# CederGroupHub/chgnet

Measured on AMD Instinct MI355X. Metric: structures/s (energy+force+stress) on batched ~50-atom crystals, higher is better.
Workload: dtype f32; 1 GPU; 1024 x LiMnO2 5x1x1 (40 atoms, sigma=0.01 frac perturbation) per GPU, task efs; structures_per_gpu=1024, atoms=40960, directed_bonds=3535504, angles=4125764, bond_graph_nodes=213755, weights=random-init 0.3.0 architecture (tests/golden/weights_seed0.npz), parallelism=structures sharded over 1 GPU(s), RCCL all-gather of energies only, process_group_ranks=1, energies_in_all_gather=1024, comm=none (single rank)

## Files before the change

chgnet_amd/csrc/engine.hip:

```cpp

#include "engine_internal.h"
#include <cstring>

namespace chgh {

template <int UNROLL>
__global__ __launch_bounds__(256) void k_stream_copy(const f32x4* __restrict__ src, f32x4* __restrict__ dst, size_t n) {
  const size_t stride = (size_t)gridDim.x * blockDim.x;
  size_t i = (size_t)blockIdx.x * blockDim.x + threadIdx.x;
  for (; i + (UNROLL - 1) * stride < n; i += UNROLL * stride) {
    f32x4 v[UNROLL];
#pragma unroll
    for (int u = 0; u < UNROLL; ++u) v[u] = __builtin_nontemporal_load(src + i + u * stride);
#pragma unroll
    for (int u = 0; u < UNROLL; ++u) __builtin_nontemporal_store(v[u], dst + i + u * stride);
  }
  for (; i < n; i += stride) dst[i] = src[i];
}

template <bool NT>
__global__ __launch_bounds__(256) void k_stream_copy_seg(const f32x4* __restrict__ src, f32x4* __restrict__ dst, size_t n) {
  constexpr size_t SEG = 1024;
  const size_t nseg = n / SEG;
  for (size_t sgm = blockIdx.x; sgm < nseg; sgm += gridDim.x) {
// ... 202 lines not shown
    const int sa = acquire_arena(eng, b, total);
    if (sa != CHG_OK) { delete b; return sa; }
  }
  carve(b, b->arena, total);
  if (h->atom_off) b->h_atom_off.assign(h->atom_off, h->atom_off + h->n_struct + 1);
  b->h_volume.resize(h->n_struct);
  for (int q = 0; q < h->n_struct; ++q) {
    const float* Lf = h->lattice + 9 * q;
    b->h_volume[q] = Lf[0] * (Lf[4] * Lf[8] - Lf[5] * Lf[7]) + Lf[1] * (Lf[5] * Lf[6] - Lf[3] * Lf[8]) + Lf[2] * (Lf[3] * Lf[7] - Lf[4] * Lf[6]);
  }
  int s = CHG_OK;
  const size_t B = b->B, N = b->N, Ed = b->Ed, Eu = b->Eu, A = b->A, Eb = b->Eb;
#define UP(field, n) if (s == CHG_OK) s = h2d(eng, b->field, h->field, (n), eng->copy_stream)
  UP(z, N); UP(atom_owner, N); UP(atom_off, B + 1); UP(frac, 3 * N); UP(lattice, 9 * B);
  UP(e_center, Ed); UP(e_nbr, Ed); UP(e_d2u, Ed); UP(e_owner, Ed); UP(e_image, 3 * Ed); UP(e_rev, Ed); UP(p_center, Ed); UP(p_nbr, Ed);
  UP(u_u2d, Eu); UP(u_bnode, Eu); UP(bn_und, Eb);
  UP(a_ctr, A); UP(a_b1c, A); UP(a_b2c, A); UP(a_d1, A); UP(a_d2, A);
#undef UP
  b->win_pending = true;
  if (s == CHG_OK && hipStreamSynchronize(eng->copy_stream) != hipSuccess) { eng->err = "chg_batch_upload: sync failed"; s = CHG_EHIP; }
  if (s != CHG_OK) { hipFree(b->arena); delete b; return s; }
  *out = b;
  return CHG_OK;
}

int chg_debug_fetch_i32(chg_engine* eng, chg_batch* b, const char* name, int32_t* dst, int64_t capacity, int64_t* n_written) {
  if (!eng || !b || !name || !dst) return CHG_EINVAL;
  if (std::strcmp(name, "wide_range") == 0) {
    if (capacity >= 1) dst[0] = b->wide_range ? 1 : 0;
    if (n_written) *n_written = capacity >= 1 ? 1 : 0;
    return CHG_OK;
  }
  if (std::strcmp(name, "route") == 0) {
    const int64_t n = std::min<int64_t>(6, std::max<int64_t>(capacity, 0));
    std::copy(b->route, b->route + n, dst);
    if (n_written) *n_written = n;
    return CHG_OK;
  }
  if (b->named_i32.empty()) register_names(b);
  auto it = b->named_i32.find(name);
  if (it == b->named_i32.end()) { eng->err = std::string("chg_debug_fetch_i32: unknown buffer ") + name; return CHG_EINVAL; }
  const size_t n = std::min<size_t>(it->second.second, (size_t)std::max<int64_t>(capacity, 0));
  TRY(ensure_windows(eng, b));
  HIP_TRY(eng, hipStreamSynchronize(eng->stream));
  if (n) HIP_TRY(eng, hipMemcpy(dst, it->second.first, n * sizeof(int32_t), hipMemcpyDeviceToHost));
  if (n_written) *n_written = (int64_t)n;
  return CHG_OK;
}

int chg_batch_update_geometry(chg_engine* eng, chg_batch* b, const float* frac, const float* lattice) {
  if (!eng || !b) return CHG_EINVAL;
  HIP_TRY(eng, hipSetDevice(eng->device));
  int s = CHG_OK;
  if (frac) s = h2d(eng, b->frac, frac, (size_t)3 * b->N);
  if (s == CHG_OK && lattice) {
    s = h2d(eng, b->lattice, lattice, (size_t)9 * b->B);
    b->h_volume.resize(b->B);
    for (int q = 0; q < b->B; ++q) {
      const float* Lf = lattice + 9 * (size_t)q;
      b->h_volume[q] = Lf[0] * (Lf[4] * Lf[8] - Lf[5] * Lf[7]) + Lf[1] * (Lf[5] * Lf[6] - Lf[3] * Lf[8]) + Lf[2] * (Lf[3] * Lf[7] - Lf[4] * Lf[6]);
    }
  }
  b->q_tables = false;
  if (s == CHG_OK) HIP_TRY(eng, hipStreamSynchronize(eng->stream));
  return s;
}

// ... 14 lines not shown
  }
  delete b;
  return CHG_OK;
}

int64_t chg_batch_device_bytes(const chg_batch* b) { return b ? (int64_t)b->arena_bytes : 0; }

int chg_predict(chg_engine* eng, chg_batch* b, uint32_t task_mask) {
  if (!eng || !b) return CHG_EINVAL;
  HIP_TRY(eng, hipSetDevice(eng->device));
  const uint32_t task = task_mask | CHG_TASK_E;
  TRY(ensure_windows(eng, b));
  if (eng->force_wide) b->wide_range = true;
  if (b->wide_range) return chgh_wide::run_predict(eng, b, task);
  if (eng->profiling || !eng->use_graphs) return run_predict(eng, b, task);
  if (b->graph_task != task) {
    if (b->graph_exec) hipGraphExecDestroy(b->graph_exec);
    b->graph_exec = nullptr;
    b->graph_task = task;
    b->eager_calls = 0;
  }
  if (!b->graph_exec && b->eager_calls++ == 0) return run_predict(eng, b, task);
  if (!b->graph_exec) {
    hipGraph_t graph = nullptr;
    HIP_TRY(eng, hipStreamBeginCapture(eng->stream, hipStreamCaptureModeThreadLocal));
    const int s = run_predict(eng, b, task);
    const hipError_t e = hipStreamEndCapture(eng->stream, &graph);
    if (s != CHG_OK) { if (graph) hipGraphDestroy(graph); return s; }
    if (e != hipSuccess) { eng->err = std::string("hipStreamEndCapture: ") + hipGetErrorString(e); return CHG_EHIP; }
    const hipError_t ei = hipGraphInstantiate(&b->graph_exec, graph, nullptr, nullptr, 0);
    hipGraphDestroy(graph);
    if (ei != hipSuccess) { b->graph_exec = nullptr; eng->err = std::string("hipGraphInstantiate: ") + hipGetErrorString(ei); return CHG_EHIP; }
    b->graph_task = task;
    std::copy(b->route, b->route + 6, b->graph_route);
  }
  HIP_TRY(eng, hipGraphLaunch(b->graph_exec, eng->stream));
  std::copy(b->graph_route, b->graph_route + 6, b->route);
  b->last_task = task;
  b->seed1_adjoints = (task & (CHG_TASK_F | CHG_TASK_S)) != 0;
  b->q_tables = b->seed1_adjoints;
  return CHG_OK;
}

int chg_engine_update_weights(chg_engine* eng, const float* weights_blob) {
  if (!eng || !weights_blob) return CHG_EINVAL;
  TRY(check_weight_range(eng, weights_blob, (size_t)eng->desc.n_weights));
  HIP_TRY(eng, hipSetDevice(eng->device));
  HIP_TRY(eng, hipMemcpyAsync(eng->d_weights, weights_blob, sizeof(float) * (size_t)eng->desc.n_weights, hipMemcpyHostToDevice, eng->stream));
  TRY(build_images(eng));
  HIP_TRY(eng, hipStreamSynchronize(eng->stream));
  return CHG_OK;
}

int chg_batch_all_gather_energy(chg_engine* eng, chg_batch* b, chg_comm* comm, int64_t width, float* table) {
  if (!eng || !b || !comm || !table || width < b->B) return CHG_EINVAL;
  if (b->last_task == 0) { eng->err = "chg_batch_all_gather_energy: run chg_predict on this batch first"; return CHG_EINVAL; }
  HIP_TRY(eng, hipSetDevice(eng->device));
  int32_t nranks = 1, comm_dev = -1;
  float* stage = nullptr;
  if (chg_comm_info(comm, nullptr, &nranks, &comm_dev) == CHG_OK && comm_dev != eng->device) {
    eng->err = "chg_batch_all_gather_energy: the communicator belongs to device " + std::to_string(comm_dev) + ", the engine to device " + std::to_string(eng->device);
    return CHG_EINVAL;
  }
  if (chg_comm_info(comm, nullptr, &nranks, nullptr) != CHG_OK || chg_comm_reserve(comm, width * (int64_t)(nranks + 1), &stage) != CHG_OK) {
    eng->err = std::string("chg_batch_all_gather_energy: ") + chg_comm_last_error(comm);
    return CHG_EHIP;
  }
  hipStream_t st = eng->stream;
  HIP_TRY(eng, hipMemsetAsync(stage, 0, sizeof(float) * (size_t)width, st));
  HIP_TRY(eng, hipMemcpyAsync(stage, b->energy, sizeof(float) * (size_t)b->B, hipMemcpyDeviceToDevice, st));
// ... 234 lines not shown
```

chgnet_amd/csrc/engine_internal.h:

```cpp
#pragma once

#include "chgnet_hip.h"

#include <hip/hip_runtime.h>

#include <algorithm>
#include <cmath>
#include <cstdint>
#include <cstdio>
#include <cstdlib>
#include <cstring>
#include <functional>
#include <map>
#include <mutex>
#include <string>
#include <unordered_map>
#include <vector>

#include "mfma_tile.h"
#include "mfma_split.h"
#include "kernels_conv.h"
#include "kernels_angle_w.h"
#include "kernels_angle_blk.h"
#include "kernels_embed.h"
// ... 18 lines not shown
};

struct ErrText {
  static std::unordered_map<const ErrText*, std::string>& texts() {
    thread_local std::unordered_map<const ErrText*, std::string> t;
    return t;
  }
  std::string& slot() const { return texts()[this]; }
  ErrText& operator=(const std::string& v) { slot() = v; return *this; }
  ErrText& operator=(const char* v) { slot() = v; return *this; }
  operator std::string() const { return slot(); }
  const char* c_str() const { return slot().c_str(); }
  ~ErrText() { texts().erase(this); }
};
inline std::string operator+(const char* a, const ErrText& b) { return std::string(a) + std::string(b); }
inline std::string operator+(const std::string& a, const ErrText& b) { return a + std::string(b); }
inline std::string operator+(const ErrText& a, const char* b) { return std::string(a) + b; }
inline std::string operator+(const ErrText& a, const std::string& b) { return std::string(a) + b; }

struct ProfEntry { std::string label; int64_t launches = 0; double ms = 0.0; };
struct PendingEvent { int entry; hipEvent_t start, stop; };

struct chg_engine {
  int device = 0;
  hipStream_t stream = nullptr;
  chg_model_desc desc{};
  float* d_weights = nullptr;
  Weights w{};
  float* d_images = nullptr;
  const float* p_elem = nullptr;
  const float* img_ac_fwd[2][MAX_CONV] = {};
  const float* img_ac_bwd_rm[MAX_CONV] = {};
  const float* img_angle[2][2 * MAX_CONV] = {};
  ErrText err;
  hipEvent_t t0 = nullptr, t1 = nullptr;
  bool profiling = false;
  std::vector<ProfEntry> prof;
  std::map<std::string, int> prof_index;
  std::vector<PendingEvent> pending;
  std::vector<hipEvent_t> event_pool;
  hipStream_t copy_stream = nullptr;
  std::mutex pool_mu;
  std::vector<std::pair<char*, size_t>> arena_pool;
  std::vector<std::pair<char*, size_t>> work_pool;
  std::vector<int> work_kind;
  bool use_graphs = true;
  bool force_wide = false;
  char* scratch = nullptr;
  size_t scratch_bytes = 0, scratch_wanted = 0;
  char* h_stage = nullptr;
  size_t h_stage_bytes = 0;
  char* h_out = nullptr;
  size_t h_out_bytes = 0;
  int num_cus = 256;
  bool spec_builds = true;
  int last_N = 0, last_Ed = 0, last_A = 0, last_Eb = 0;
  double last_r_atom = 0.0, last_r_bond = 0.0;
  long n_spec_builds = 0, n_spec_overflows = 0, n_cell_builds = 0, n_cell_fallbacks = 0;
  int graph_search = 0;
  int cell_min_atoms = 2048;
  size_t memory_limit = 0;
};

struct Train2;

struct chg_batch {
// ... 2 lines not shown
  size_t arena_bytes = 0;
  int *z, *atom_owner, *atom_off, *e_center, *e_nbr, *e_d2u, *e_owner, *e_rev, *p_center, *p_nbr, *u_u2d, *u_bnode, *bn_und, *a_ctr, *a_b1c, *a_b2c, *a_d1, *a_d2;
  float *frac, *lattice, *e_image;
  float* cart;
  f32x4 *ev, *eu;
  float *hb0, *wag, *wbgc;
  float* atom[MAX_CONV + 1];
  float* hbc[MAX_CONV + 1];
  float* ang[MAX_CONV];
  float* Pl[MAX_CONV];
  float* Ql[MAX_CONV];
  float* Rl[2 * MAX_CONV];
  float* Sl[2 * MAX_CONV];
  float* agg_l[MAX_CONV];
  float* aggB_l[MAX_CONV];
  float* GP_l[MAX_CONV];
  float* GR_l[2 * MAX_CONV];
  float* GS_l[2 * MAX_CONV];
  float* zsave_l[2 * MAX_CONV] = {};
  float *energy, *site_energy, *site_raw, *magmom, *crystal_fea, *force, *virial, *volume;
  float *Ga, *GA, *Gb, *Gwag, *Gwbgc, *Gang, *GQ, *Gagg, *Grk, *Gu;
  WinIndex win{};
  int *win_tmp = nullptr, *win_scan = nullptr;
  int win_grid = 64;
  bool win_built = false;
  bool canonical = false;
  bool win_index_ready = false;
  int win_team = 0;
  int blk_cap = 0;
  bool blk_ready = false;
  int *blk_a = nullptr, *blk_b1c = nullptr, *blk_b2c = nullptr, *blk_ctr = nullptr, *blk_desc = nullptr, *blk_tiles = nullptr;
  bool win_pending = false;
  bool zsave_now = false;
  int32_t route[6] = {}, graph_route[6] = {};
  size_t addr_span = 0;
  int p_table_done = -1;
  float *zero1, *zero1_end, *zero2, *zero2_end;
  float* zero2_keep_end = nullptr;
  uint32_t last_task = 0;
  bool seed1_adjoints = false;
  hipGraphExec_t graph_exec = nullptr;
  uint32_t graph_task = 0;
  int eager_calls = 0;
  std::map<std::string, std::pair<const float*, size_t>> named;
  std::map<std::string, std::pair<const int*, size_t>> named_i32;
  char* train_arena = nullptr;
  size_t train_bytes = 0;
  std::vector<int> h_atom_off;
  std::vector<double> h_volume;
  char* t2_arena = nullptr;
  size_t t2_bytes = 0;
  struct Train2* t2 = nullptr;
  float* t_mcot = nullptr;
  float h_g_b3 = 0.f;
  bool q_tables = false;
  bool wide_range = false;
  bool t_has_mcot = false;
  float *t_grad = nullptr, *t_cot = nullptr, *t_tmp = nullptr , *t_dumpG = nullptr, *t_dumpH = nullptr, *t_dumpZ = nullptr, *t_Xb = nullptr, *t_Xa = nullptr,
        *t_ro = nullptr;
};

#define HIP_TRY(eng, expr)                                                                          \
  do {                                                                                              \
    hipError_t _e = (expr);                                                                         \
    if (_e != hipSuccess) {                                                                         \
      (eng)->err = std::string(#expr) + ": " + hipGetErrorString(_e);                               \
      return CHG_EHIP;                                                                              \
// ... 135 lines not shown
```

chgnet_amd/csrc/engine_predict.hip:

```cpp
#include "engine_internal.h"

#include "kernels_geom.h"
#include "kernels_angle_fa.h"
#include "kernels_chain.h"

namespace chgh {


struct Cursor {
  const float* base;
  size_t pos = 0;
  const float* take(size_t n) {
    pos += (4 - pos % 4) % 4;
    const float* p = base + pos;
    pos += n;
    return p;
  }
};

void take_gated_tail(Cursor& c, GatedW& g, const float*& w2c_t, const float*& w2g_t) {
  g.w2c = c.take(D * D); g.b2c = c.take(D); g.w2g = c.take(D * D); g.b2g = c.take(D);
  w2c_t = c.take(D * D); w2g_t = c.take(D * D);
}
void take_ln(Cursor& c, GatedW& g) {
  g.ln1_g = c.take(D); g.ln1_b = c.take(D); g.ln2_g = c.take(D); g.ln2_b = c.take(D);
}

size_t layout_weights(const float* base, int L, Weights& w) {
  Cursor c{base};
  w.atomref = c.take(94); w.emb = c.take(94 * D);
  w.freq_ag = c.take(NRAD); w.freq_bg = c.take(NRAD); w.freq_ang = c.take(NFREQ);
  w.w_bond_emb = c.take(D * NRAD); w.w_wag = c.take(D * NRAD); w.w_wbg = c.take(D * NRAD); w.w_ang_emb = c.take(D * NANG);
  for (int l = 0; l < L; ++l) {
    ACW& a = w.ac[l];
    a.w_cn = c.take(4 * D * D); a.w_bond = c.take(2 * D * D); a.b1 = c.take(2 * D); a.q_bias = c.take(2 * D); a.q_shift = c.take(D);
    take_gated_tail(c, a.g, a.w2c_t, a.w2g_t);
    take_ln(c, a.g);
// ... 137 lines not shown
  hipLaunchKernelGGL((k_rows_gemm_multi<K, SMALL_GEMM_COLS>), dim3(grid_for(m.max_rows, 4 * eng->num_cus), blocks), dim3(BLOCK),
                     (rows_gemm_lds<K, SMALL_GEMM_COLS, (K == 128 ? 2 : 1)>()), eng->stream, m.g);
  HIP_TRY(eng, hipGetLastError());
  return CHG_OK;
}
static bool small_rows(int rows) { return rows > 0 && rows <= SMALL_GEMM_ROWS; }

int zero(chg_engine* eng, void* p, size_t bytes) {
  if (bytes == 0) return CHG_OK;
  LaunchScope ls(eng, "memset");
  HIP_TRY(eng, hipMemsetAsync(p, 0, bytes, eng->stream));
  return CHG_OK;
}





static bool addr32_mode(const chg_batch* b) {
  constexpr size_t HARD = (size_t)1 << 32;
  static const int forced = [] { const char* e = std::getenv("CHGNET_ADDR_MODE"); return e ? std::atoi(e) : 0; }();
  static const size_t limit = [] { const char* e = std::getenv("CHGNET_ADDR32_MAX_BYTES"); return e ? (size_t)std::strtoull(e, nullptr, 10) : HARD; }();
  if (b->addr_span == 0 || b->addr_span >= HARD || forced == 64) return false;
  return forced == 32 || b->addr_span < limit;
}

int build_images(chg_engine* eng) {
  const int L = eng->desc.n_conv;
  constexpr size_t AF = ac_fwd_image_floats(), AB = ac_bwd_rm_image_floats();
  constexpr size_t BF = AngleLds<true, false>::tiles, BB = AngleLds<true, true>::tiles, UF = AngleLds<false, false>::tiles,
                   UB = AngleLds<false, true>::tiles;
  static_assert(AF % 4 == 0 && AB % 4 == 0 && BF % 4 == 0 && BB % 4 == 0 && UF % 4 == 0 && UB % 4 == 0, "images are copied in 16-byte units");
  constexpr size_t PE = (size_t)94 * 4 * D;
  const size_t total = (size_t)L * (2 * AF + AB) + (size_t)(L - 1) * (BF + BB + UF + UB) + PE;
  if (!eng->d_images) {
    HIP_TRY(eng, hipMalloc(&eng->d_images, total * sizeof(float)));
    HIP_TRY(eng, hipMemsetAsync(eng->d_images, 0, total * sizeof(float), eng->stream));
  }
  float* at = eng->d_images;
  auto take = [&](size_t n) { float* p = at; at += n; return p; };
  for (int l = 0; l < L; ++l) {
    AtomConvArgs a{};
    a.gw = eng->w.ac[l].g; a.w_bond = eng->w.ac[l].w_bond;
    for (int qb = 0; qb < 2; ++qb) {
      a.q_bias = qb ? eng->w.ac[l].q_bias : nullptr;
      float* img = take(AF);
      eng->img_ac_fwd[qb][l] = img;
      hipLaunchKernelGGL(k_atomconv_image<>, dim3(1), dim3(BLOCK), 0, eng->stream, a, img);
    }
    float* img = take(AB);
    eng->img_ac_bwd_rm[l] = img;
    hipLaunchKernelGGL(k_atomconv_image_rm, dim3(1), dim3(BLOCK), 0, eng->stream, a, img);
  }
  for (int l = 0; l + 1 < L; ++l) {
    const BCW& bc = eng->w.bc[l];
    const AUW& au = eng->w.au[l];
    float* img;
    eng->img_angle[0][l] = img = take(BF);
    hipLaunchKernelGGL((k_angle_image<true, false>), dim3(1), dim3(BLOCK), 0, eng->stream, bc.w_ang, bc.g, img);
    eng->img_angle[1][l] = img = take(BB);
    hipLaunchKernelGGL((k_angle_image<true, true>), dim3(1), dim3(BLOCK), 0, eng->stream, bc.w_ang, bc.g, img);
    eng->img_angle[0][L + l] = img = take(UF);
    hipLaunchKernelGGL((k_angle_image<false, false>), dim3(1), dim3(BLOCK), 0, eng->stream, au.w_ang, au.g, img);
    eng->img_angle[1][L + l] = img = take(UB);
    hipLaunchKernelGGL((k_angle_image<false, true>), dim3(1), dim3(BLOCK), 0, eng->stream, au.w_ang, au.g, img);
  }
  {
    float* tab = take(PE);
    eng->p_elem = tab;
    const ACW& w0 = eng->w.ac[0];
    TRY(rows_gemm_out2(eng, "gemm_Pelem", eng->w.emb, nullptr, w0.w_cn, w0.w_cn + 2 * D * D, w0.b1, tab, 4 * D, 94));
  }
  HIP_TRY(eng, hipGetLastError());
  return CHG_OK;
}

static bool tiny_batch(const chg_batch* b) {
  static const bool on = [] { const char* e = std::getenv("CHGNET_TINY_FUSE"); return !e || std::atoi(e) != 0; }();
  return on && b->N <= SMALL_GEMM_ROWS && b->Ed <= (1 << 18) && b->A <= (1 << 19);
}

static RowsGemm atomconv_p_problem(chg_engine* eng, chg_batch* b, int l) {
  const ACW& w = eng->w.ac[l];
  return RowsGemm{b->atom[l], D, nullptr, w.w_cn, w.b1, nullptr, 0, b->Pl[l], 4 * D, nullptr, b->N, 0, w.w_cn + 2 * D * D, 0, 2 * D, 0, 0};
}

int atomconv_tables(chg_engine* eng, chg_batch* b, int l) {
  const ACW& w = eng->w.ac[l];
  if (b->p_table_done == l) return CHG_OK;
  return rows_gemm_out2(eng, "gemm_P", b->atom[l], nullptr, w.w_cn, w.w_cn + 2 * D * D, w.b1, b->Pl[l], 4 * D, b->N);
}

int atomconv_q_table(chg_engine* eng, chg_batch* b, int l) {
  const ACW& w = eng->w.ac[l];
  float* Q = b->Ql[l];
  if (b->Eu == 0) return CHG_OK;
  TRY(rows_gemm(eng, "gemm_Q", 64, 128, b->hb0, D, nullptr, w.w_bond, b->A > 0 ? w.q_bias : nullptr, nullptr, 0, Q, 2 * D, nullptr, b->Eu, 0));
  if (b->Eb > 0 && b->hbc[l] != b->hbc[0])
    TRY(rows_gemm(eng, "gemm_Qnode", 64, 128, b->hbc[l], D, nullptr, w.w_bond, nullptr, nullptr, 0, Q, 2 * D, b->bn_und, b->Eb, 0));
  return CHG_OK;
}

AtomConvArgs atomconv_args(chg_engine* eng, chg_batch* b, int l) {
  AtomConvArgs a{};
// ... 312 lines not shown
        cb.term(p, b->GR_l[L + l], 4 * D, nullptr, w.au[l].w_bij_t, 2 * D);
        cb.term(p, b->GR_l[L + l] + 2 * D, 4 * D, nullptr, w.au[l].w_bij_t + 2 * D * D, 2 * D);
        p.Y1 = b->Gb; p.y1_idx = b->bn_und; p.ldy1 = D;
      }
      p.add = b->Gb; p.add_idx = b->bn_und; p.lda = D;
      cb.out(p, w.bc[l].w_out_t, nullptr, b->Gagg, D, D);
      if (au) {
        ChainProb& q = cb.add(b->N);
        cb.term(q, b->GS_l[L + l], 2 * D, nullptr, w.au[l].w_ctr_t, 2 * D);
        q.add = b->Ga; q.lda = D; q.Y1 = b->Ga; q.ldy1 = D;
      }
      TRY(launch_chain(eng, "chain_Bt", cb));
    }
    TRY((launch_angle<true, true>(eng, "bondconv_bwd", b, angle_args(b, l, b->ang[l], w.bc[l].w_ang, w.bc[l].g, nullptr))));
    {
      ChainBuilder cb;
      ChainProb& p = cb.add(b->N);
      cb.term(p, b->GS_l[l], 2 * D, nullptr, w.bc[l].w_ctr_t, 2 * D);
      cb.term(p, b->GP_l[l + 1], 4 * D, nullptr, w.ac[l + 1].w_cn_t, 2 * D);
      cb.term(p, b->GP_l[l + 1] + 2 * D, 4 * D, nullptr, w.ac[l + 1].w_cn_t + 2 * D * D, 2 * D);
      p.add = b->Ga; p.lda = D; p.Y1 = b->Ga; p.ldy1 = D;
      cb.out(p, w.ac[l].w_out_t, nullptr, b->GA, D, D);
      ChainProb& q = cb.add(b->Eb);
      cb.term(q, b->GR_l[l], 4 * D, nullptr, w.bc[l].w_bij_t, 2 * D);
      cb.term(q, b->GR_l[l] + 2 * D, 4 * D, nullptr, w.bc[l].w_bij_t + 2 * D * D, 2 * D);
      q.add = b->Gb; q.add_idx = b->bn_und; q.lda = D; q.Y1 = b->Gb; q.y1_idx = b->bn_und; q.ldy1 = D;
      TRY(launch_chain(eng, "chain_At", cb));
    }
    TRY(atomconv_bwd_kernel(eng, b, l));
  }
  return CHG_OK;
}

int run_predict(chg_engine* eng, chg_batch* b, uint32_t task) {
  const Weights& w = eng->w;
  const int L = b->L;
  const bool want_f = task & CHG_TASK_F, want_s = task & CHG_TASK_S, want_m = task & CHG_TASK_M;
  const bool want_grad = want_f || want_s;
  hipStream_t st = eng->stream;

  const bool tiny = tiny_batch(b);
  b->zsave_now = want_grad;
  const size_t zero_bytes = (size_t)((char*)(want_grad ? b->zero2_end : b->zero1_end) - (char*)b->zero1);
  b->p_table_done = -1;
  if (tiny) {
    PrologueArgs a{};
    a.frac = b->frac; a.lattice = b->lattice; a.atom_owner = b->atom_owner; a.z = b->z; a.n_atoms = b->N;
    a.e_center = b->e_center; a.e_nbr = b->e_nbr; a.e_owner = b->e_owner; a.e_image = b->e_image; a.n_edges = b->Ed;
    a.cart = b->cart; a.ev = b->ev; a.eu = b->eu; a.emb = w.emb; a.atom0 = b->atom[0];
    a.p_elem = b->Ed > 0 ? eng->p_elem : nullptr; a.P0 = b->Pl[0];
    a.zero_begin = reinterpret_cast<f32x4*>(b->zero1); a.zero_n = zero_bytes / sizeof(f32x4);
    LaunchScope ls(eng, "prologue");
    hipLaunchKernelGGL(k_prologue, dim3(std::min<unsigned>(4 * eng->num_cus, g1(std::max<int64_t>(b->Ed, (int64_t)b->N * D)).x)), dim3(256), 0, st, a);
    if (a.p_elem) b->p_table_done = 0;
  } else {
    LaunchScope ls(eng, "cart");
    hipLaunchKernelGGL(k_cart, g1(b->N), dim3(256), 0, st, b->frac, b->lattice, b->atom_owner, b->cart, b->N);
  }
  if (b->Ed > 0) {
    if (!tiny) { LaunchScope ls(eng, "edge_geom");
      hipLaunchKernelGGL(k_edge_geom, g1(b->Ed), dim3(256), 0, st, b->cart, b->lattice, b->e_center, b->e_nbr, b->e_image, b->e_owner, b->ev, b->eu, b->Ed); }
    if (tiny) {
      EmbedAllArgs ea{bond_embed_args(eng, b), angle_embed_args(eng, b), grid_for(b->Eu, 2 * eng->num_cus),
                      b->Eb > 0 ? grid_for(b->Eb, 2 * eng->num_cus) : 0, b->A > 0 ? grid_for(b->A, EMBED_GRID_MULT * eng->num_cus) : 0};
      LaunchScope ls(eng, "embed_fwd");
      hipLaunchKernelGGL(k_embed_all<false>, dim3(ea.g_bond1 + ea.g_bond2 + ea.g_angle), dim3(BLOCK), bond_embed_lds(), st, ea);
    } else { LaunchScope ls(eng, "bond_embed_fwd");
      hipLaunchKernelGGL((k_bond_embed_fwd_o4<1>), dim3(grid_for(b->Eu, 2 * eng->num_cus)), dim3(BLOCK), bond_embed_lds(), st, bond_embed_args(eng, b));
      if (b->Eb > 0)
        hipLaunchKernelGGL((k_bond_embed_t<false, false, 2>), dim3(grid_for(b->Eb, 2 * eng->num_cus)), dim3(BLOCK), bond_embed_lds(), st, bond_embed_args(eng, b)); }
  }
  if (b->A > 0 && !(tiny && b->Ed > 0)) {
    LaunchScope ls(eng, "angle_embed_fwd");
    hipLaunchKernelGGL((k_angle_embed_fwd_o4<0>), dim3(grid_for(b->A, EMBED_GRID_MULT * eng->num_cus)), dim3(BLOCK), angle_embed_lds(), st, angle_embed_args(eng, b));
  }
  if (!tiny) { LaunchScope ls(eng, "atom_embed");
    hipLaunchKernelGGL(k_atom_embed, g1((int64_t)b->N * (D / 4)), dim3(256), 0, st, b->z, w.emb, b->atom[0], b->N); }
  HIP_TRY(eng, hipGetLastError());

  if (!tiny) TRY(zero(eng, b->zero1, zero_bytes));
  static const bool chain_on = [] { const char* e = std::getenv("CHGNET_TINY_CHAIN"); return !e || std::atoi(e) != 0; }();
  const bool chained = tiny && chain_on && L >= 2 && b->Ed > 0 && b->A > 0 && b->Eb > 0 && b->p_table_done == 0;
  b->route[0] = tiny;
  b->route[1] = chained;
  b->route[2] = want_grad && b->zsave_l[0] && (b->win_built || b->win_team > 0);
  b->route[3] = b->win_built;
  b->route[4] = b->win_team > 0;
  b->route[5] = addr32_mode(b);
  if (chained) {
    TRY(forward_tiny(eng, b, want_grad, want_m));
  } else {
  for (int l = 0; l < L - 1; ++l) {
    TRY(atomconv_fwd(eng, b, l, want_grad));
    if (b->A > 0) {
      TRY(bondconv_fwd(eng, b, l));
      if (l < L - 2) TRY(angleupd_fwd(eng, b, l));
    }
  }
  if (want_m) {
    LaunchScope ls(eng, "magmom");
    hipLaunchKernelGGL(k_magmom, dim3(wave_grid(eng, b->N)), dim3(256), 0, st, b->atom[L - 1], w.site_w, w.site_b, b->magmom, b->N);
  }
  TRY(atomconv_fwd(eng, b, L - 1, want_grad));
  }

  {
    ReadoutArgs r{};
    r.atom = b->atom[L]; r.atom_owner = b->atom_owner; r.z = b->z; r.n_atoms = b->N;
    r.ln_g = w.ro_ln_g; r.ln_b = w.ro_ln_b; r.w0 = w.mlp_w0; r.b0 = w.mlp_b0; r.w1 = w.mlp_w1; r.b1 = w.mlp_b1;
    r.w2 = w.mlp_w2; r.b2 = w.mlp_b2; r.w3 = w.mlp_w3; r.b3 = w.mlp_b3; r.atomref = w.atomref;
    r.has_composition = eng->desc.has_composition; r.n_hidden = eng->desc.n_mlp_hidden;
    r.site_energy = b->site_energy; r.site_raw = b->site_raw; r.crystal_fea = b->crystal_fea;
    r.Ga = want_grad ? b->Ga : nullptr;
    const int tiles16 = (b->N + TILE_ROWS - 1) / TILE_ROWS;
    r.wpb = std::max(1, std::min(WAVES, (tiles16 + eng->num_cus - 1) / eng->num_cus));
    LaunchScope ls(eng, "readout");
    hipLaunchKernelGGL(k_readout<false>, dim3(grid_for(b->N, eng->num_cus, r.wpb * TILE_ROWS)), dim3(BLOCK), readout_lds(), st, r);
    HIP_TRY(eng, hipGetLastError());
  }

  if (want_grad) {
    if (chained) {
      TRY(reverse_tiny(eng, b));
    } else {
    TRY(atomconv_bwd(eng, b, L - 1));
    for (int l = L - 2; l >= 0; --l) {
      if (b->A > 0) {
        if (l < L - 2) TRY(angleupd_bwd(eng, b, l));
        TRY(bondconv_bwd(eng, b, l));
      }
      TRY(atomconv_bwd(eng, b, l));
    }
    }
    if (b->Ed > 0) {
      if (tiny) {
        EmbedAllArgs ea{bond_embed_args(eng, b), angle_embed_args(eng, b), grid_for(b->Eu, 2 * eng->num_cus),
                        b->Eb > 0 ? grid_for(b->Eb, 2 * eng->num_cus) : 0, b->A > 0 ? grid_for(b->A, EMBED_GRID_MULT * eng->num_cus) : 0};
        LaunchScope ls(eng, "embed_bwd");
        hipLaunchKernelGGL(k_embed_all<true>, dim3(ea.g_bond1 + ea.g_bond2 + ea.g_angle), dim3(BLOCK), bond_embed_lds(), st, ea);
      } else { LaunchScope ls(eng, "bond_embed_bwd");
        hipLaunchKernelGGL((k_bond_embed_t<true, false, 1>), dim3(grid_for(b->Eu, 2 * eng->num_cus)), dim3(BLOCK), bond_embed_lds(), st, bond_embed_args(eng, b));
        if (b->Eb > 0)
          hipLaunchKernelGGL((k_bond_embed_t<true, false, 2>), dim3(grid_for(b->Eb, 2 * eng->num_cus)), dim3(BLOCK), bond_embed_lds(), st, bond_embed_args(eng, b)); }
      if (b->A > 0 && !tiny) {
        LaunchScope ls(eng, "angle_embed_bwd");
        hipLaunchKernelGGL((k_angle_embed_t<true>), dim3(grid_for(b->A, EMBED_GRID_MULT * eng->num_cus)), dim3(BLOCK), angle_embed_lds(), st, angle_embed_args(eng, b));
      }
      ForceArgs f{};
      f.ev = b->ev; f.eu = b->eu; f.Gu = b->Gu; f.Grk = b->Grk;
      f.e_center = b->e_center; f.e_d2u = b->e_d2u; f.e_owner = b->e_owner; f.e_rev = b->e_rev; f.u_u2d = b->u_u2d;
      f.n_edges = b->Ed; f.force = b->force; f.virial = b->virial;
      LaunchScope ls(eng, "edge_force");
      hipLaunchKernelGGL(k_edge_force, g1(b->Ed, EF_EDGES_PER_BLOCK), dim3(256), 0, st, f);
    }
    HIP_TRY(eng, hipGetLastError());
  }
// ... 211 lines not shown
  if ((s = set_lds(eng, k_rows_gemm<128, SMALL_GEMM_COLS, 2>, (rows_gemm_lds<128, SMALL_GEMM_COLS, 2>())))) return s;
  if ((s = set_lds(eng, (k_rows_gemm<64, 128, 2>), (rows_gemm_lds<64, 128, 2>())))) return s;
  if ((s = set_lds(eng, (k_rows_gemm<128, 64, 2>), (rows_gemm_lds<128, 64, 2>())))) return s;
  if ((s = set_lds(eng, k_atomconv_fwd<FWD_WAVES>, (atomconv_lds<FWD_WAVES, false, true>())))) return s;
  if ((s = set_lds(eng, k_atomconv_bwd<false>, acb_fused_lds()))) return s;
  if ((s = set_lds(eng, k_angleupd_fwd_a<>, angle_fa_lds()))) return s;
  if ((s = set_lds(eng, (k_atomconv_fwd<FWD_WAVES, true>), (atomconv_lds<FWD_WAVES, false, true>())))) return s;
  if ((s = set_lds(eng, (k_atomconv_bwd<false, true>), acb_fused_lds()))) return s;
  if ((s = set_lds(eng, k_angleupd_fwd_a<true>, angle_fa_lds()))) return s;
  if ((s = set_lds(eng, (k_angle_bwd_w<true, false, false, true>), angle_w_lds<true>()))) return s;
  if ((s = set_lds(eng, (k_angle_bwd_w<true, false, true, true>), angle_w_lds<true>()))) return s;
  if ((s = set_lds(eng, (k_angle_bwd_w<false, false, false, true>), angle_w_lds<false>()))) return s;
  if ((s = set_lds(eng, (k_angle<true, false, WAVES, false, true>), angle_lds<true>()))) return s;
  if ((s = set_lds(eng, k_angle_bwd_blk<true>, angle_blk_lds<true>()))) return s;
  if ((s = set_lds(eng, k_angle_bwd_blk<false>, angle_blk_lds<false>()))) return s;
  if ((s = set_lds(eng, k_angle_bwd_w<true>, angle_w_lds<true>()))) return s;
  if ((s = set_lds(eng, k_angle_bwd_w<false>, angle_w_lds<false>()))) return s;
  if ((s = set_lds(eng, (k_angle_bwd_w<true, true>), angle_w_lds<true>()))) return s;
  if ((s = set_lds(eng, (k_angle_bwd_w<true, false, true>), angle_w_lds<true>()))) return s;
  if ((s = set_lds(eng, (k_angle_bwd_w<true, true, true>), angle_w_lds<true>()))) return s;
  if ((s = set_lds(eng, (k_angle_bwd_w<false, true>), angle_w_lds<false>()))) return s;
  if ((s = set_lds(eng, k_angle<true, false>, angle_lds<true>()))) return s;
  if ((s = set_lds(eng, k_angle<true, true>, (angle_lds<true, WAVES, true>())))) return s;
  if ((s = set_lds(eng, k_angle<false, true>, (angle_lds<false, WAVES, true>())))) return s;
  if ((s = set_lds(eng, k_angle<false, false, FWD_WAVES>, (angle_lds<false, FWD_WAVES>())))) return s;
  if ((s = set_lds(eng, k_readout<false>, readout_lds()))) return s;
  if ((s = set_lds(eng, (k_bond_embed_t<false, false, 2>), bond_embed_lds()))) return s;
  if ((s = set_lds(eng, (k_bond_embed_t<true, false, 1>), bond_embed_lds()))) return s;
  if ((s = set_lds(eng, (k_bond_embed_t<true, false, 2>), bond_embed_lds()))) return s;
  if ((s = set_lds(eng, k_angle_embed_fwd_o4<0>, angle_embed_lds()))) return s;
  if ((s = set_lds(eng, k_bond_embed_fwd_o4<1>, bond_embed_lds()))) return s;
  if ((s = set_lds(eng, k_angle_embed_t<true>, angle_embed_lds()))) return s;
  if ((s = set_lds(eng, k_rows_chain, chain_lds()))) return s;
  if ((s = set_lds(eng, k_embed_all<false>, bond_embed_lds()))) return s;
  if ((s = set_lds(eng, k_embed_all<true>, bond_embed_lds()))) return s;
  return CHG_OK;
}


}
```

Measured before the change: 40710 structures/s.

## Merge per-row linear layers into multi-output MFMA kernels for forward and reverse

Result: no change. 40810 structures/s, median of 6 (+0.2%).

```diff
diff --git a/chgnet_amd/csrc/engine.hip b/chgnet_amd/csrc/engine.hip
--- a/chgnet_amd/csrc/engine.hip
+++ b/chgnet_amd/csrc/engine.hip
@@ -258,7 +258,7 @@
     return CHG_OK;
   }
   if (std::strcmp(name, "route") == 0) {
-    const int64_t n = std::min<int64_t>(6, std::max<int64_t>(capacity, 0));
+    const int64_t n = std::min<int64_t>(chg_batch::N_ROUTE, std::max<int64_t>(capacity, 0));
     std::copy(b->route, b->route + n, dst);
     if (n_written) *n_written = n;
     return CHG_OK;
@@ -339,10 +339,10 @@
     hipGraphDestroy(graph);
     if (ei != hipSuccess) { b->graph_exec = nullptr; eng->err = std::string("hipGraphInstantiate: ") + hipGetErrorString(ei); return CHG_EHIP; }
     b->graph_task = task;
-    std::copy(b->route, b->route + 6, b->graph_route);
+    std::copy(b->route, b->route + chg_batch::N_ROUTE, b->graph_route);
   }
   HIP_TRY(eng, hipGraphLaunch(b->graph_exec, eng->stream));
-  std::copy(b->graph_route, b->graph_route + 6, b->route);
+  std::copy(b->graph_route, b->graph_route + chg_batch::N_ROUTE, b->route);
   b->last_task = task;
   b->seed1_adjoints = (task & (CHG_TASK_F | CHG_TASK_S)) != 0;
   b->q_tables = b->seed1_adjoints;
diff --git a/chgnet_amd/csrc/engine_internal.h b/chgnet_amd/csrc/engine_internal.h
--- a/chgnet_amd/csrc/engine_internal.h
+++ b/chgnet_amd/csrc/engine_internal.h
@@ -74,6 +74,8 @@
   const float* img_ac_fwd[2][MAX_CONV] = {};
   const float* img_ac_bwd_rm[MAX_CONV] = {};
   const float* img_angle[2][2 * MAX_CONV] = {};
+  struct RowsImg { const float *cn, *cn_t, *ctr, *ctr_t, *bij, *bij_t, *out, *out_t; };
+  RowsImg img_rows_ac[MAX_CONV] = {}, img_rows_bc[MAX_CONV] = {}, img_rows_au[MAX_CONV] = {};
   ErrText err;
   hipEvent_t t0 = nullptr, t1 = nullptr;
   bool profiling = false;
@@ -142,7 +144,8 @@
   int *blk_a = nullptr, *blk_b1c = nullptr, *blk_b2c = nullptr, *blk_ctr = nullptr, *blk_desc = nullptr, *blk_tiles = nullptr;
   bool win_pending = false;
   bool zsave_now = false;
-  int32_t route[6] = {}, graph_route[6] = {};
+  static constexpr int N_ROUTE = 7;
+  int32_t route[N_ROUTE] = {}, graph_route[N_ROUTE] = {};
   size_t addr_span = 0;
   int p_table_done = -1;
   float *zero1, *zero1_end, *zero2, *zero2_end;
diff --git a/chgnet_amd/csrc/engine_predict.hip b/chgnet_amd/csrc/engine_predict.hip
--- a/chgnet_amd/csrc/engine_predict.hip
+++ b/chgnet_amd/csrc/engine_predict.hip
@@ -3,6 +3,7 @@
 #include "kernels_geom.h"
 #include "kernels_angle_fa.h"
 #include "kernels_chain.h"
+#include "kernels_rows.h"
 
 namespace chgh {
 
@@ -206,7 +207,9 @@
                    UB = AngleLds<false, true>::tiles;
   static_assert(AF % 4 == 0 && AB % 4 == 0 && BF % 4 == 0 && BB % 4 == 0 && UF % 4 == 0 && UB % 4 == 0, "images are copied in 16-byte units");
   constexpr size_t PE = (size_t)94 * 4 * D;
-  const size_t total = (size_t)L * (2 * AF + AB) + (size_t)(L - 1) * (BF + BB + UF + UB) + PE;
+  constexpr size_t RA = 4 * RM_IMG64 + 2 * RM_IMG128 + 2 * RM_IMG64, RU = 2 * RM_IMG64 + RM_IMG128 + 4 * RM_IMG64 + 2 * RM_IMG128,
+                   RB = RU + 2 * RM_IMG64;
+  const size_t total = (size_t)L * (2 * AF + AB) + (size_t)(L - 1) * (BF + BB + UF + UB) + PE + (size_t)L * RA + (size_t)(L - 1) * (RB + RU);
   if (!eng->d_images) {
     HIP_TRY(eng, hipMalloc(&eng->d_images, total * sizeof(float)));
     HIP_TRY(eng, hipMemsetAsync(eng->d_images, 0, total * sizeof(float), eng->stream));
@@ -244,6 +247,31 @@
     eng->p_elem = tab;
     const ACW& w0 = eng->w.ac[0];
     TRY(rows_gemm_out2(eng, "gemm_Pelem", eng->w.emb, nullptr, w0.w_cn, w0.w_cn + 2 * D * D, w0.b1, tab, 4 * D, 94));
+  }
+  {
+    auto images = [&](const float* W, int K, int n) {
+      float* first = take((size_t)n * D * K);
+      for (int q = 0; q < n; ++q)
+        hipLaunchKernelGGL(k_rows_image, dim3(1), dim3(BLOCK), 0, eng->stream, W + (size_t)q * D * K, D, K, first + (size_t)q * D * K);
+      return (const float*)first;
+    };
+    for (int l = 0; l < L; ++l) {
+      const ACW& a = eng->w.ac[l];
+      chg_engine::RowsImg& r = eng->img_rows_ac[l];
+      r = chg_engine::RowsImg{};
+      r.cn = images(a.w_cn, D, 4); r.cn_t = images(a.w_cn_t, 2 * D, 2); r.out = images(a.w_out, D, 1); r.out_t = images(a.w_out_t, D, 1);
+    }
+    for (int l = 0; l + 1 < L; ++l) {
+      const BCW& bc = eng->w.bc[l];
+      const AUW& au = eng->w.au[l];
+      chg_engine::RowsImg& rb = eng->img_rows_bc[l];
+      rb = chg_engine::RowsImg{};
+      rb.ctr = images(bc.w_ctr, D, 2); rb.ctr_t = images(bc.w_ctr_t, 2 * D, 1); rb.bij = images(bc.w_bij, D, 4); rb.bij_t = images(bc.w_bij_t, 2 * D, 2);
+      rb.out = images(bc.w_out, D, 1); rb.out_t = images(bc.w_out_t, D, 1);
+      chg_engine::RowsImg& ru = eng->img_rows_au[l];
+      ru = chg_engine::RowsImg{};
+      ru.ctr = images(au.w_ctr, D, 2); ru.ctr_t = images(au.w_ctr_t, 2 * D, 1); ru.bij = images(au.w_bij, D, 4); ru.bij_t = images(au.w_bij_t, 2 * D, 2);
+    }
   }
   HIP_TRY(eng, hipGetLastError());
   return CHG_OK;
@@ -622,6 +650,149 @@
   return CHG_OK;
 }
 
+static int rows_merge_mode() {
+  static const int mode = [] {
+    const char* e = std::getenv("CHGNET_ROWS_MERGE");
+    const int v = e ? std::atoi(e) : 1;
+    return v == 0 ? 0 : v == 2 ? 1 : v == 3 ? 2 : 3;
+  }();
+  return mode;
+}
+
+struct MergeBuilder {
+  RowsMerge p{};
+  explicit MergeBuilder(int rows) { p.rows = rows; }
+  void term(const float* X, int ldx, const float* img, int K) { p.t[p.nterms++] = ChainTerm{X, nullptr, img, ldx, K}; }
+  void out(const float* img, const float* bias, int bias_blocks, float* Y, int ldy, int nblocks) {
+    for (int q = 0; q < nblocks; ++q)
+      p.o[p.nouts++] = RmOut{img + (size_t)q * RM_IMG64, (bias && q < bias_blocks) ? bias + q * D : nullptr, Y + q * D, ldy};
+  }
+  void add(const float* rows, const int* idx) { p.add = rows; p.idx = idx; p.lda = D; }
+  void store(float* Y1) { p.Y1 = Y1; p.ldy1 = D; }
+};
+
+int launch_rows_merge(chg_engine* eng, const char* label, MergeBuilder& mb) {
+  RowsMerge& p = mb.p;
+  if (p.rows <= 0) return CHG_OK;
+  const int K = p.nterms ? p.t[0].K : D;
+  for (int t = 1; t < p.nterms; ++t)
+    if (p.t[t].K != K) { eng->err = "rows_merge: terms of different widths"; return CHG_EINVAL; }
+  const int ny = (p.nouts + 3) / 4;
+  p.outs_per_block = ny ? (p.nouts + ny - 1) / ny : 0;
+  const size_t lds = rows_merge_lds(p);
+  if (lds > RM_LDS_CAP || (ny > 1 && p.Y1 == p.add)) { eng->err = "rows_merge: unsupported problem"; return CHG_EINVAL; }
+  const int ntiles = (p.rows + BLOCK_ROWS - 1) / BLOCK_ROWS;
+  const int gx = rm_phases(p.nterms) > 1 ? ntiles : grid_for(p.rows, std::max(8, 2 * eng->num_cus / std::max(ny, 1)));
+  LaunchScope ls(eng, label);
+  const dim3 grid(gx, std::max(ny, 1));
+  if (K == D) hipLaunchKernelGGL(k_rows_merge<D>, grid, dim3(BLOCK), lds, eng->stream, p);
+  else hipLaunchKernelGGL(k_rows_merge<2 * D>, grid, dim3(BLOCK), lds, eng->stream, p);
+  HIP_TRY(eng, hipGetLastError());
+  return CHG_OK;
+}
+
+int forward_merged(chg_engine* eng, chg_batch* b, bool want_grad, bool want_m) {
+  const Weights& w = eng->w;
+  const int L = b->L;
+  const bool angles = b->A > 0;
+  for (int l = 0; l < L; ++l) {
+    if (b->p_table_done != l) {
+      MergeBuilder mb(b->N);
+      mb.add(b->atom[l], nullptr);
+      mb.out(eng->img_rows_ac[l].cn, w.ac[l].b1, 2, b->Pl[l], 4 * D, 4);
+      TRY(launch_rows_merge(eng, "rows_atom_f", mb));
+      b->p_table_done = l;
+    }
+    TRY(atomconv_fwd_kernel(eng, b, l, want_grad));
+    {
+      MergeBuilder mb(b->N);
+      mb.term(b->agg_l[l], D, eng->img_rows_ac[l].out, D);
+      mb.p.bias1 = w.ac[l].b_out;
+      mb.add(b->atom[l], nullptr);
+      mb.store(b->atom[l + 1]);
+      if (l < L - 1) {
+        if (angles) mb.out(eng->img_rows_bc[l].ctr, w.bc[l].b1, 2, b->Sl[l], 2 * D, 2);
+        mb.out(eng->img_rows_ac[l + 1].cn, w.ac[l + 1].b1, 2, b->Pl[l + 1], 4 * D, 4);
+        if (angles && l < L - 2) mb.out(eng->img_rows_au[l].ctr, w.au[l].b1, 2, b->Sl[L + l], 2 * D, 2);
+      }
+      TRY(launch_rows_merge(eng, "rows_atom_f", mb));
+      if (l < L - 1) b->p_table_done = l + 1;
+    }
+    if (l == L - 1) break;
+    if (angles) {
+      if (l == 0) {
+        MergeBuilder mb(b->Eb);
+        mb.add(b->hbc[0], nullptr);
+        mb.out(eng->img_rows_bc[0].bij, nullptr, 0, b->Rl[0], 4 * D, 4);
+        TRY(launch_rows_merge(eng, "rows_bond_f", mb));
+      }
+      TRY((launch_angle<true, false>(eng, "bondconv_fwd", b, angle_args(b, l, b->ang[l], w.bc[l].w_ang, w.bc[l].g, b->aggB_l[l]))));
+      MergeBuilder mb(b->Eb);
+      mb.term(b->aggB_l[l], D, eng->img_rows_bc[l].out, D);
+      mb.p.bias1 = w.bc[l].b_out;
+      mb.add(b->hbc[l], nullptr);
+      mb.store(b->hbc[l + 1]);
+      if (l < L - 2) {
+        mb.out(eng->img_rows_au[l].bij, nullptr, 0, b->Rl[L + l], 4 * D, 4);
+        mb.out(eng->img_rows_bc[l + 1].bij, nullptr, 0, b->Rl[l + 1], 4 * D, 4);
+      }
+      TRY(launch_rows_merge(eng, "rows_bond_f", mb));
+      if (l < L - 2)
+        TRY((launch_angle<false, false, FWD_WAVES>(eng, "angleupd_fwd", b, angle_args(b, L + l, b->ang[l], w.au[l].w_ang, w.au[l].g, b->ang[l + 1]))));
+    }
+    if (l == L - 2 && want_m) {
+      LaunchScope ls(eng, "magmom");
+      hipLaunchKernelGGL(k_magmom, dim3(wave_grid(eng, b->N)), dim3(256), 0, eng->stream, b->atom[L - 1], w.site_w, w.site_b, b->magmom, b->N);
+    }
+  }
+  return CHG_OK;
+}
+
+int reverse_merged(chg_engine* eng, chg_batch* b) {
+  const int L = b->L;
+  const bool angles = b->A > 0;
+  auto gr_terms = [&](MergeBuilder& mb, int slot, const chg_engine::RowsImg& im) {
+    mb.term(b->GR_l[slot], 4 * D, im.bij_t, 2 * D);
+    mb.term(b->GR_l[slot] + 2 * D, 4 * D, im.bij_t + RM_IMG128, 2 * D);
+  };
+  for (int l = L - 1; l >= 0; --l) {
+    if (angles && l < L - 1) {
+      const bool au = l < L - 2;
+      if (au) TRY((launch_angle<false, true>(eng, "angleupd_bwd", b, angle_args(b, L + l, b->ang[l], eng->w.au[l].w_ang, eng->w.au[l].g, nullptr))));
+      {
+        MergeBuilder mb(b->Eb);
+        if (au) { gr_terms(mb, L + l, eng->img_rows_au[l]); mb.store(b->Gb); }
+        mb.add(b->Gb, b->bn_und);
+        mb.out(eng->img_rows_bc[l].out_t, nullptr, 0, b->Gagg, D, 1);
+        TRY(launch_rows_merge(eng, "rows_bond_b", mb));
+      }
+      TRY((launch_angle<true, true>(eng, "bondconv_bwd", b, angle_args(b, l, b->ang[l], eng->w.bc[l].w_ang, eng->w.bc[l].g, nullptr))));
+      {
+        MergeBuilder mb(b->Eb);
+        gr_terms(mb, l, eng->img_rows_bc[l]);
+        mb.add(b->Gb, b->bn_und);
+        mb.store(b->Gb);
+        TRY(launch_rows_merge(eng, "rows_bond_b", mb));
+      }
+    }
+    {
+      MergeBuilder mb(b->N);
+      if (l < L - 1) {
+        if (angles && l < L - 2) mb.term(b->GS_l[L + l], 2 * D, eng->img_rows_au[l].ctr_t, 2 * D);
+        if (angles) mb.term(b->GS_l[l], 2 * D, eng->img_rows_bc[l].ctr_t, 2 * D);
+        mb.term(b->GP_l[l + 1], 4 * D, eng->img_rows_ac[l + 1].cn_t, 2 * D);
+        mb.term(b->GP_l[l + 1] + 2 * D, 4 * D, eng->img_rows_ac[l + 1].cn_t + RM_IMG128, 2 * D);
+        mb.store(b->Ga);
+      }
+      mb.add(b->Ga, nullptr);
+      mb.out(eng->img_rows_ac[l].out_t, nullptr, 0, b->GA, D, 1);
+      TRY(launch_rows_merge(eng, "rows_atom_b", mb));
+    }
+    TRY(atomconv_bwd_kernel(eng, b, l));
+  }
+  return CHG_OK;
+}
+
 int run_predict(chg_engine* eng, chg_batch* b, uint32_t task) {
   const Weights& w = eng->w;
   const int L = b->L;
@@ -677,8 +848,12 @@
   b->route[3] = b->win_built;
   b->route[4] = b->win_team > 0;
   b->route[5] = addr32_mode(b);
+  const int merged = (!tiny && L >= 2 && b->Ed > 0) ? rows_merge_mode() : 0;
+  b->route[6] = merged;
   if (chained) {
     TRY(forward_tiny(eng, b, want_grad, want_m));
+  } else if (merged & 1) {
+    TRY(forward_merged(eng, b, want_grad, want_m));
   } else {
   for (int l = 0; l < L - 1; ++l) {
     TRY(atomconv_fwd(eng, b, l, want_grad));
@@ -712,6 +887,8 @@
   if (want_grad) {
     if (chained) {
       TRY(reverse_tiny(eng, b));
+    } else if (merged & 2) {
+      TRY(reverse_merged(eng, b));
     } else {
     TRY(atomconv_bwd(eng, b, L - 1));
     for (int l = L - 2; l >= 0; --l) {
@@ -989,6 +1166,8 @@
   if ((s = set_lds(eng, k_bond_embed_fwd_o4<1>, bond_embed_lds()))) return s;
   if ((s = set_lds(eng, k_angle_embed_t<true>, angle_embed_lds()))) return s;
   if ((s = set_lds(eng, k_rows_chain, chain_lds()))) return s;
+  if ((s = set_lds(eng, k_rows_merge<D>, RM_LDS_CAP))) return s;
+  if ((s = set_lds(eng, k_rows_merge<2 * D>, RM_LDS_CAP))) return s;
   if ((s = set_lds(eng, k_embed_all<false>, bond_embed_lds()))) return s;
   if ((s = set_lds(eng, k_embed_all<true>, bond_embed_lds()))) return s;
   return CHG_OK;
diff --git a/chgnet_amd/csrc/kernels_rows.h b/chgnet_amd/csrc/kernels_rows.h
--- /dev/null
+++ b/chgnet_amd/csrc/kernels_rows.h
@@ -0,0 +1,188 @@
+#pragma once
+
+#include "kernels_chain.h"
+
+namespace chg {
+
+constexpr int RM_TERMS = 4, RM_OUTS = 8, RM_PHASE_TERMS = 2;
+constexpr int RM_IMG64 = D * D, RM_IMG128 = 2 * D * D;
+struct RmOut {
+  const float* img;
+  const float* bias;
+  float* Y;
+  int ldy;
+};
+struct RowsMerge {
+  int rows, nterms, nouts;
+  int outs_per_block;
+  ChainTerm t[RM_TERMS];
+  const float* bias1;
+  const float* add;
+  const int* idx;
+  int lda;
+  float* Y1;
+  int ldy1;
+  RmOut o[RM_OUTS];
+};
+
+__host__ __device__ constexpr int rm_w1_floats(int nterms, int k0) { return nterms == 0 ? 0 : (nterms == 1 && k0 == D) ? RM_IMG64 : RM_PHASE_TERMS * RM_IMG128; }
+__host__ __device__ constexpr int rm_phases(int nterms) { return (nterms + RM_PHASE_TERMS - 1) / RM_PHASE_TERMS; }
+inline size_t rows_merge_lds(const RowsMerge& p) {
+  return sizeof(float) * ((size_t)rm_w1_floats(p.nterms, p.nterms ? p.t[0].K : D) + (size_t)p.outs_per_block * (RM_IMG64 + D) + D + (size_t)WAVES * TILE_ROWS * CH_TS);
+}
+constexpr size_t RM_LDS_CAP = 120 * 1024;
+
+__device__ __forceinline__ void rm_copy16(float* dst, const float* __restrict__ src, int n16, int tid) {
+  for (int i0 = tid; i0 < n16; i0 += 4 * BLOCK) {
+    f32x4 v[4];
+#pragma unroll
+    for (int u = 0; u < 4; ++u)
+      if (i0 + u * BLOCK < n16) v[u] = reinterpret_cast<const f32x4*>(src)[i0 + u * BLOCK];
+#pragma unroll
+    for (int u = 0; u < 4; ++u)
+      if (i0 + u * BLOCK < n16) reinterpret_cast<f32x4*>(dst)[i0 + u * BLOCK] = v[u];
+  }
+}
+
+static __global__ __launch_bounds__(BLOCK) void k_rows_image(const float* W, int F, int K, float* out) {
+  stage_split<false>(reinterpret_cast<h16x8*>(out), W, F, K, threadIdx.x, BLOCK);
+}
+
+template <int K>
+__device__ __forceinline__ void rm_transpose(f32x4 (&x)[K / 16], const ChainX& r, float* T, int lane, int j, int g) {
+  constexpr int LPR = K / 4, RPS = 64 / LPR, NV = TILE_ROWS / RPS;
+  const int sub = lane / LPR, t = lane % LPR;
+#pragma unroll
+  for (int h = 0; h < K / D; ++h) {
+    if ((t >> 4) == h) {
+#pragma unroll
+      for (int it = 0; it < NV; ++it) *reinterpret_cast<f32x4*>(T + (RPS * it + sub) * CH_TS + 4 * (t & 15)) = r.v[it];
+    }
+    __builtin_amdgcn_wave_barrier();
+    f32x4 xh[VT];
+    read_dl<VT>(T + j * CH_TS, g, xh);
+#pragma unroll
+    for (int f = 0; f < VT; ++f) x[VT * h + f] = xh[f];
+    __builtin_amdgcn_wave_barrier();
+  }
+}
+
+template <int K>
+__global__ __launch_bounds__(BLOCK) CHG_TWO_WAVES void k_rows_merge(RowsMerge p) {
+  extern __shared__ __attribute__((aligned(16))) float smem[];
+  constexpr int KT = K / 16;
+  const int nob_max = p.outs_per_block;
+  float* W1 = smem;
+  float* W2 = W1 + rm_w1_floats(p.nterms, K);
+  float* b2s = W2 + nob_max * RM_IMG64;
+  float* b1s = b2s + nob_max * D;
+  float* tiles = b1s + D;
+  const int tid = threadIdx.x, wave = tid >> 6, lane = tid & 63, j = lane & 15, g = lane >> 4;
+  const int ob0 = blockIdx.y * nob_max;
+  const int nob = min(nob_max, p.nouts - ob0);
+  const int nphases = rm_phases(p.nterms);
+  auto stage_phase = [&](int ph) {
+#pragma unroll
+    for (int s = 0; s < RM_PHASE_TERMS; ++s) {
+      const int t = RM_PHASE_TERMS * ph + s;
+      if (t < p.nterms) rm_copy16(W1 + s * RM_IMG128, p.t[t].W, K * (D / 4), tid);
+    }
+  };
+  for (int q = 0; q < nob; ++q) {
+    rm_copy16(W2 + q * RM_IMG64, p.o[ob0 + q].img, RM_IMG64 / 4, tid);
+    if (tid < D) b2s[q * D + tid] = p.o[ob0 + q].bias ? p.o[ob0 + q].bias[tid] : 0.f;
+  }
+  if (tid < D) b1s[tid] = p.bias1 ? p.bias1[tid] : 0.f;
+  if (nphases == 1) stage_phase(0);
+  __syncthreads();
+  float* T = tiles + wave * TILE_ROWS * CH_TS;
+  const int sub4 = lane >> 4, t4 = lane & 15;
+  const int ntiles = (p.rows + BLOCK_ROWS - 1) / BLOCK_ROWS;
+  int tb, te;
+  tile_range(ntiles, tb, te);
+  auto rows_of = [&](int tile, int& nvalid, int& rr_) {
+    const int row0 = tile * BLOCK_ROWS + wave * TILE_ROWS;
+    nvalid = min(TILE_ROWS, p.rows - row0);
+    rr_ = nvalid > 0 ? row0 + min(j, nvalid - 1) : 0;
+  };
+  auto issue_terms = [&](int ph, int rr_, ChainX& r0, ChainX& r1) {
+    const int t0 = RM_PHASE_TERMS * ph;
+    chain_x_issue<K>(r0, p.t[t0], rr_, lane);
+    if (t0 + 1 < p.nterms) chain_x_issue<K>(r1, p.t[t0 + 1], rr_, lane);
+  };
+  for (int tile = tb; tile < te; ++tile) {
+    int nvalid, rr_;
+    rows_of(tile, nvalid, rr_);
+    const int row0 = tile * BLOCK_ROWS + wave * TILE_ROWS;
+    const bool active = nvalid > 0;
+    const int map_row = p.idx ? p.idx[rr_] : rr_;
+    f32x4 av[TILE_ROWS / 4];
+    int orow[TILE_ROWS / 4];
+#pragma unroll
+    for (int it = 0; it < TILE_ROWS / 4; ++it) {
+      orow[it] = __shfl(map_row, 4 * it + sub4);
+      av[it] = zero4();
+      if (active && p.add) av[it] = *reinterpret_cast<const f32x4*>(p.add + (size_t)orow[it] * p.lda + 4 * t4);
+    }
+    f32x4 acc[VT];
+    read_dl<VT>(b1s, g, acc);
+    for (int ph = 0; ph < nphases; ++ph) {
+      if (nphases > 1) {
+        __syncthreads();
+        stage_phase(ph);
+        __syncthreads();
+      }
+      if (active) {
+        const bool two = RM_PHASE_TERMS * ph + 1 < p.nterms;
+        ChainX r0, r1;
+        issue_terms(ph, rr_, r0, r1);
+        f32x4 x0[KT], x1[KT];
+        rm_transpose<K>(x0, r0, T, lane, j, g);
+        if (two) rm_transpose<K>(x1, r1, T, lane, j, g);
+        gemm_split<KT, VT, true>(acc, reinterpret_cast<const h16x8*>(W1), D, x0, j, g);
+        if (two) gemm_split<KT, VT, true>(acc, reinterpret_cast<const h16x8*>(W1 + RM_IMG128), D, x1, j, g);
+      }
+    }
+    if (!active) continue;
+    write_dl<VT>(T + j * CH_TS, g, acc);
+    __builtin_amdgcn_wave_barrier();
+#pragma unroll
+    for (int it = 0; it < TILE_ROWS / 4; ++it) {
+      av[it] += *reinterpret_cast<const f32x4*>(T + (4 * it + sub4) * CH_TS + 4 * t4);
+      asm volatile("" : "+v"(av[it]));
+    }
+    const bool store1 = p.Y1 && blockIdx.y == 0;
+#pragma unroll
+    for (int it = 0; it < TILE_ROWS / 4; ++it) {
+      const int rr = 4 * it + sub4;
+      *reinterpret_cast<f32x4*>(T + rr * CH_TS + 4 * t4) = av[it];
+      if (store1 && rr < nvalid) *reinterpret_cast<f32x4*>(p.Y1 + (size_t)orow[it] * p.ldy1 + 4 * t4) = av[it];
+    }
+    if (nob <= 0) continue;
+    __builtin_amdgcn_wave_barrier();
+    f32x4 x2[VT];
+    read_dl<VT>(T + j * CH_TS, g, x2);
+    __builtin_amdgcn_wave_barrier();
+    SplitRow<VT / 2> s2;
+    split_row<VT, true>(s2, x2);
+    for (int q = 0; q < nob; ++q) {
+      const RmOut& o = p.o[ob0 + q];
+      f32x4 acc2[VT];
+      read_dl<VT>(b2s + q * D, g, acc2);
+      gemm_split4<VT / 2, true>(acc2, reinterpret_cast<const h16x8*>(W2 + q * RM_IMG64), D, s2, 0, j, g);
+      write_dl<VT>(T + j * CH_TS, g, acc2);
+      __builtin_amdgcn_wave_barrier();
+      f32x4 ov[TILE_ROWS / 4];
+#pragma unroll
+      for (int it = 0; it < TILE_ROWS / 4; ++it) ov[it] = *reinterpret_cast<const f32x4*>(T + (4 * it + sub4) * CH_TS + 4 * t4);
+#pragma unroll
+      for (int it = 0; it < TILE_ROWS / 4; ++it) {
+        const int rr = 4 * it + sub4;
+        if (rr < nvalid) *reinterpret_cast<f32x4*>(o.Y + (size_t)(row0 + rr) * o.ldy + 4 * t4) = ov[it];
+      }
+      __builtin_amdgcn_wave_barrier();
+    }
+  }
+}
+
+}
```
